# uc-vision/taichi-splatting

Hardware: AMD Instinct MI355X
Metric: fwd+bwd Msplats/s (higher is better)
Workload: dtype f32; 1 GPU; config D: 6000000 random 3D gaussians, 2048x2048, SH deg 3, tile 16, fwd+bwd (render_gaussians, loss=image.sum()); n_gaussians=6000000, tile_size=16, sh_degree=3, mode=single, parallelism=single GPU

## Files before the change

### include/mi355_splat.h

```cpp
#ifndef MI355_SPLAT_H
#define MI355_SPLAT_H

#include <stddef.h>
#include <stdint.h>

#ifdef __cplusplus
extern "C" {
#endif

#define MS_VERSION 500
#define MS_ABI_GENERATION(version) ((version) / 100)

enum { MS_F32 = 0, MS_F64 = 1 };

enum {
  MS_ERR_BAD_ARG = -1,
  MS_ERR_UNSUPPORTED = -2,
  MS_ERR_TMP_TOO_SMALL = -3,
  MS_ERR_ABI = -4
};

typedef struct ms_raster_config {
  int32_t tile_size;
  int32_t antialias;
// ... 134 lines not shown
  uint32_t abi_version;
  int64_t n;
  int64_t k_capacity;
  int32_t image_w, image_h;
  int32_t dtype;
  int32_t f;
  int32_t sh_degree;
  int32_t depth16;
  int32_t tile_row_begin, tile_row_end;
  int32_t projected_input;
  int32_t mapper;
  int32_t split_long_runs;
  int32_t split_seg_len;
  double near_plane, far_plane, blur_cov, clamp_margin;
  ms_raster_config raster;
} ms_frame_desc;

typedef struct ms_frame_layout {
  size_t keep_n_bytes, scratch_n_bytes, keep_k_bytes, scratch_k_bytes;
  size_t points7, depth, colours, points7_f32, camera_position, counters, tile_ranges;
  size_t sorted_keys, order, counts, cum, ordered_points, tmp_n;
  size_t overlap_to_point;
  size_t keys, values, keys_sorted, tmp_k;
  size_t splat_rows;
  size_t split_scratch;
} ms_frame_layout;

typedef struct ms_frame_inputs {
  uint32_t struct_size;
  uint32_t reserved;
  const void *position, *log_scaling, *rotation, *alpha_logit, *feature, *T_camera_world, *projection;
  const void *points7, *depth, *colours;
  int32_t* longest_run_host;
  void* colours_ready_event;
} ms_frame_inputs;

enum { MS_BACKWARD_ALL = 0, MS_BACKWARD_GAUSSIANS = 1, MS_BACKWARD_RASTER = 2 };

typedef struct ms_frame_grads {
  uint32_t struct_size;
// ... 107 lines not shown
```

### taichi_splatting_amd/_lib.py

```python
from __future__ import annotations

import ctypes
from ctypes import c_int, c_int32, c_int64, c_double, c_float, c_void_p, c_size_t, c_char_p, POINTER
import os
from pathlib import Path
import subprocess
from typing import Optional

import torch

PACKAGE_DIR = Path(__file__).resolve().parent
CSRC_DIR = PACKAGE_DIR / 'csrc'
LIB_PATH = Path(os.environ.get('MS_SPLAT_LIB') or PACKAGE_DIR / 'libmi355_splat.so')

MS_F32, MS_F64 = 0, 1
BACKWARD_ALL, BACKWARD_GAUSSIANS, BACKWARD_RASTER = 0, 1, 2
BOUNDARY_AXIS_SIGMA, BOUNDARY_COVARIANCE = 0, 1
MAPPER_DIRECT, MAPPER_PRESORT = 0, 1
ABI_VERSION = 500
MOMENT_ROW = 16
SPLAT_ROW = 16

_lib: Optional[ctypes.CDLL] = None

# ... 20 lines not shown
    self.struct_size = ctypes.sizeof(type(self))
    if hasattr(self, 'abi_version'):
      self.abi_version = ABI_VERSION


class FrameDescC(_SizedStructure):
  _fields_ = [
    ('struct_size', ctypes.c_uint32), ('abi_version', ctypes.c_uint32),
    ('n', c_int64), ('k_capacity', c_int64),
    ('image_w', c_int32), ('image_h', c_int32),
    ('dtype', c_int32), ('f', c_int32), ('sh_degree', c_int32), ('depth16', c_int32),
    ('tile_row_begin', c_int32), ('tile_row_end', c_int32),
    ('projected_input', c_int32), ('mapper', c_int32), ('split_long_runs', c_int32), ('split_seg_len', c_int32),
    ('near_plane', c_double), ('far_plane', c_double), ('blur_cov', c_double), ('clamp_margin', c_double),
    ('raster', RasterConfigC),
  ]


class FrameLayoutC(ctypes.Structure):
  _fields_ = [(name, c_size_t) for name in (
    'keep_n_bytes', 'scratch_n_bytes', 'keep_k_bytes', 'scratch_k_bytes',
    'points7', 'depth', 'colours', 'points7_f32', 'camera_position', 'counters', 'tile_ranges',
    'sorted_keys', 'order', 'counts', 'cum', 'ordered_points', 'tmp_n',
    'overlap_to_point',
    'keys', 'values', 'keys_sorted', 'tmp_k',
    'splat_rows', 'split_scratch')]


class FrameInputsC(_SizedStructure):
  _fields_ = [('struct_size', ctypes.c_uint32), ('reserved', ctypes.c_uint32)] + [(name, c_void_p) for name in (
    'position', 'log_scaling', 'rotation', 'alpha_logit', 'feature', 'T_camera_world', 'projection',
    'points7', 'depth', 'colours', 'longest_run_host', 'colours_ready_event')]


class FrameGradsC(_SizedStructure):
  _fields_ = [
    ('struct_size', ctypes.c_uint32), ('reserved', ctypes.c_uint32),
    ('image', c_void_p), ('grad_image', c_void_p),
    ('extra_points7', c_void_p), ('extra_depth', c_void_p), ('extra_colours', c_void_p),
    ('moments', c_void_p), ('deterministic', c_int32), ('stage', c_int32), ('fixed_exp', c_void_p),
    ('grad_points7', c_void_p), ('grad_colours', c_void_p),
# ... 159 lines not shown
```

### taichi_splatting_amd/csrc/frame.hip

```cpp
#include <cstdlib>
#include <cstring>
#include "common.h"
#include "frame_internal.h"
#include "raster_common.h"

namespace ms {

struct FrameGeom {
  int w_pad, h_pad, tiles_wide, tiles_high, num_tiles, tile_bits, row_begin, row_end;
  size_t es;
};

static FrameGeom frame_geom(const ms_frame_desc* d) {
  FrameGeom g;
  const int ts = d->raster.tile_size;
  g.tiles_wide = (d->image_w + ts - 1) / ts;
  g.tiles_high = (d->image_h + ts - 1) / ts;
  g.w_pad = g.tiles_wide * ts;
  g.h_pad = g.tiles_high * ts;
  g.num_tiles = g.tiles_wide * g.tiles_high;
  int bits = 1;
  while ((1ll << bits) < (long long)g.num_tiles) ++bits;
  g.tile_bits = bits;
  g.row_begin = d->tile_row_begin < 0 ? 0 : d->tile_row_begin;
// ... 24 lines not shown
  if (d->depth16) {
    const FrameGeom g = frame_geom(d);
    if (g.num_tiles > 65536) { set_error("%s: use_depth16 keys hold a 16 bit tile id: too many tiles", who); return MS_ERR_BAD_ARG; }
  }
  return 0;
}

static bool frame_uses_rows(const ms_frame_desc* d) {
  static const bool on = [] { const char* e = getenv("MS_SPLAT_ROWS"); return e && e[0] == '1'; }();
  return on && !d->projected_input && d->n > 0 && raster_uses_splat_rows(&d->raster, d->f, d->dtype);
}

static bool frame_uses_split(const ms_frame_desc* d) {
  return d->split_long_runs != 0 && d->n > 0 && d->k_capacity > 0 && raster_uses_splat_rows(&d->raster, d->f, d->dtype);
}
static SplitParams frame_split_params(const ms_frame_desc* d) {
  return split_params(d->raster.tile_size, d->split_long_runs, d->split_seg_len);
}

static int check_inputs(const ms_frame_inputs* in, const char* who) {
  if (!in) { set_error("%s: inputs are null", who); return MS_ERR_BAD_ARG; }
  if (in->struct_size != sizeof(ms_frame_inputs)) {
    set_error("%s: ms_frame_inputs of another ABI (struct_size %u, this library: %u)", who, in->struct_size, (unsigned)sizeof(ms_frame_inputs));
    return MS_ERR_ABI;
  }
  return 0;
}

static int check_grads(const ms_frame_grads* g, const char* who) {
  if (!g) { set_error("%s: grads are null", who); return MS_ERR_BAD_ARG; }
// ... 23 lines not shown
  L->splat_rows = keep_n.take(frame_uses_rows(d) ? n * SPLAT_ROW * sizeof(float) : 0);
  L->keep_n_bytes = keep_n.off;

  L->sorted_keys = scratch_n.take(n * 4);
  L->order = scratch_n.take(n * 4);
  L->counts = scratch_n.take(n * 4);
  L->cum = scratch_n.take((n + 1) * 4);
  L->ordered_points = scratch_n.take(n * 7 * 4);
  L->points7_f32 = scratch_n.take(d->dtype == MS_F64 ? n * 7 * 4 : 0);
  const size_t t1 = sort_tmp_size(d->n, 4, true), t2 = scan_tmp_size(d->n);
  L->tmp_n = scratch_n.take(t1 > t2 ? t1 : t2);
  L->scratch_n_bytes = scratch_n.off;

  L->overlap_to_point = keep_k.take(k * 4);
  L->split_scratch = keep_k.take(frame_uses_split(d) ? split_scratch_bytes(d->k_capacity, d->raster.tile_size, frame_split_params(d)) : 0);
  L->keep_k_bytes = keep_k.off;

  L->keys = scratch_k.take(k * 8);
  L->values = scratch_k.take(k * 4);
  L->keys_sorted = scratch_k.take(k * 8);
  L->tmp_k = scratch_k.take(sort_tmp_size(d->k_capacity, 8));
  L->scratch_k_bytes = scratch_k.off;
}

template <typename T>
__global__ void __launch_bounds__(256)
frame_prepare_kernel(int32_t* __restrict__ counters, int32_t capacity, const T* __restrict__ Tcw, T* __restrict__ cam_out,
                     int32_t* __restrict__ ranges, int64_t range_words) {
  const int64_t i = (int64_t)blockIdx.x * blockDim.x + threadIdx.x;
  if (i < range_words) ranges[i] = 0;
// ... 221 lines not shown
      const int64_t strip_tiles = (int64_t)(g.row_end > g.row_begin ? g.row_end - g.row_begin : 0) * g.tiles_wide;
      tile_depth_sort_launch(ranges + 2 * first_tile, strip_tiles, keys_sorted, o2p, keys, s, counters + 3, in->longest_run_host);
    }
  }
  MS_CHECK_LAUNCH();

  const void* points7 = d.projected_input ? in->points7 : (const void*)(kn + L.points7);
  const void* colours = d.sh_degree >= 0 ? (const void*)(kn + L.colours) : (d.projected_input ? in->colours : in->feature);
  MS_CHECK_ARG(d.n == 0 || colours != nullptr, "colours are null");
  SplitScratch split{};
  const bool cut = frame_uses_split(desc) && keep_k != nullptr;
  if (cut) split = split_scratch_carve(kk + L.split_scratch, d.k_capacity, d.raster.tile_size, frame_split_params(desc));
  if (in->colours_ready_event) MS_CHECK_HIP(hipStreamWaitEvent(s, (hipEvent_t)in->colours_ready_event, 0));
  return raster_fwd_launch(points7, colours, frame_uses_rows(desc) ? (const float*)(kn + L.splat_rows) : nullptr, ranges, o2p,
                           d.image_w, d.image_h, d.f, &d.raster, out_image, out_alpha, out_visibility, g.row_begin, g.row_end,
                           d.dtype, stream, cut ? &split : nullptr, in->longest_run_host);
}

extern "C" int ms_frame_backward(const ms_frame_desc* desc, const ms_frame_inputs* in, void* keep_n, void* keep_k,
                                 const ms_frame_grads* gr, void* stream) {
  MS_TRY(check_desc(desc, "ms_frame_backward"));
  MS_TRY(check_inputs(in, "ms_frame_backward"));
  MS_TRY(check_grads(gr, "ms_frame_backward"));
  MS_CHECK_ARG(in && keep_n && gr, "null pointer");
  MS_CHECK_ARG(gr->stage == MS_BACKWARD_GAUSSIANS || (gr->image && gr->grad_image), "null image / grad_image");
  const ms_frame_desc& d = *desc;
  const FrameGeom g = frame_geom(desc);
  ms_frame_layout L;
  frame_layout(desc, &L);
  hipStream_t s = (hipStream_t)stream;
  char* kn = (char*)keep_n;
// ... 20 lines not shown
    MS_CHECK_ARG(!d.projected_input, "projected input has no per-gaussian backward");
    if (gr->gather_world > 0)
      MS_CHECK_ARG(gr->gather_rows && gr->gather_slots && gr->gather_route && gr->boundary_stride >= 7 + d.f && d.dtype == MS_F32,
                   "gathered boundary gradients: rows, slots, route, boundary_stride >= 7 + f, float32");
    else
      MS_CHECK_ARG(gr->grad_points7 != nullptr, "grad_points7 is null");
  } else if (moments) {
    MS_CHECK_ARG(gr->moments != nullptr, "moments is null");
    SplitScratch split{};
    const bool cut = frame_uses_split(desc) && keep_k != nullptr;
    if (cut) split = split_scratch_carve(kk + L.split_scratch, d.k_capacity, d.raster.tile_size, frame_split_params(desc));
    MS_TRY(raster_bwd_moments_launch(points7, colours, ranges, o2p, gr->image, gr->grad_image, d.image_w, d.image_h, &d.raster,
                                     (float*)gr->moments, gr->deterministic, gr->fixed_exp, g.row_begin, g.row_end,
                                     gr->grad_image_broadcast, s,
                                     frame_uses_rows(desc) ? (const float*)(kn + L.splat_rows) : nullptr,
                                     cut ? &split : nullptr));
    if (raster_only)
      return moments_finalize_rezero_launch((const float*)points7, (float*)gr->moments, gr->deterministic, gr->fixed_exp,
                                            d.n, (float*)gr->grad_points7, (float*)gr->grad_colours,
                                            d.raster.compute_point_heuristic ? (float*)gr->point_heuristic : nullptr, s,
                                            gr->boundary_stride, d.projected_input && gr->stage != MS_BACKWARD_RASTER ? 0 : gr->boundary_form);
  } else {
    MS_CHECK_ARG(gr->grad_points7 || gr->grad_colours, "no gradient accumulator");
    MS_TRY(ms_raster_bwd(points7, colours, ranges, o2p, gr->image, gr->grad_image, d.image_w, d.image_h, d.f, &d.raster,
                         gr->grad_points7, gr->grad_colours, d.raster.compute_point_heuristic ? gr->point_heuristic : nullptr,
                         g.row_begin, g.row_end, d.dtype, stream));
    if (raster_only) return 0;
  }

  GaussianBwdArgs a{};
  a.dtype = d.dtype;
// ... 28 lines not shown
```

### taichi_splatting_amd/csrc/frame_internal.h

```cpp
#pragma once
#include "common.h"

namespace ms {

constexpr uint32_t CULLED_DEPTH_KEY = 0xffffffffu;

template <typename T>
__device__ inline void camera_position_solve(const T* __restrict__ m, T* __restrict__ out) {
#pragma clang fp contract(off)
  double a[4][5];
  for (int r = 0; r < 4; ++r) {
    for (int c = 0; c < 4; ++c) a[r][c] = (double)m[r * 4 + c];
    a[r][4] = r == 3 ? 1.0 : 0.0;
  }
  for (int col = 0; col < 4; ++col) {
    int piv = col;
    for (int r = col + 1; r < 4; ++r)
      if (fabs(a[r][col]) > fabs(a[piv][col])) piv = r;
    for (int c = 0; c < 5; ++c) { const double t = a[col][c]; a[col][c] = a[piv][c]; a[piv][c] = t; }
    const double inv = 1.0 / a[col][col];
    for (int c = 0; c < 5; ++c) a[col][c] *= inv;
    for (int r = 0; r < 4; ++r) {
      if (r == col) continue;
      const double fct = a[r][col];
// ... 39 lines not shown
                            uint64_t* scratch, hipStream_t s, int32_t* run_stats = nullptr, int32_t* run_host = nullptr);

int project_fwd_launch(const void* position, const void* log_scaling, const void* rotation, const void* alpha_logit,
                       const void* T_camera_world, const void* projection, int image_w, int image_h, double near_plane,
                       double far_plane, double blur_cov, double clamp_margin, double alpha_threshold, int64_t n,
                       void* out_points7, void* out_depth, int32_t* out_flag, int dtype, void* stream, float* splat_rows,
                       const void* colours_in);

int sh_fwd_inplace_launch(const void* params, const void* positions, const void* depth, const void* cam_pos,
                          int64_t n, int f, int degree, void* out, int dtype, hipStream_t s, float* splat_rows = nullptr);

bool raster_uses_splat_rows(const ms_raster_config* cfg, int f, int dtype);
int raster_fwd_launch(const void* points7, const void* features, const float* splat_rows, const int32_t* tile_ranges,
                      const int32_t* overlap_to_point, int image_w, int image_h, int f, const ms_raster_config* cfg,
                      void* out_image, void* out_alpha, void* out_visibility, int tile_row_begin, int tile_row_end,
                      int dtype, void* stream, const struct SplitScratch* split = nullptr, int32_t* long_run_word = nullptr);

int raster_bwd_moments_launch(const void* points7, const void* features, const int32_t* tile_ranges,
                              const int32_t* overlap_to_point, const void* image, const void* grad_image, int image_w,
                              int image_h, const ms_raster_config* cfg, float* moments, int deterministic,
                              const int32_t* fixed_exp, int tile_row_begin, int tile_row_end, int grad_broadcast,
                              hipStream_t s, const float* splat_rows = nullptr, const struct SplitScratch* split = nullptr);
int moments_finalize_rezero_launch(const float* points7, float* moments, int deterministic, const int32_t* fixed_exp,
                                   int64_t n, float* grad_points7, float* grad_features, float* point_heuristic,
                                   hipStream_t s, int row_stride = 0, int covariance_form = 0);

struct FastParams;
bool launch_rows_backward(const float* points7, const float* features, const int32_t* tile_ranges,
                          const int32_t* overlap_to_point, const float* image, const float* grad_image,
                          const FastParams& rp, int tile_size, bool heuristics, float* moments, const int32_t* fixed_exp,
                          hipStream_t s);

struct GaussianBwdArgs {
  int dtype;
  int64_t n;
  const void *position, *log_scaling, *rotation, *alpha_logit, *T_camera_world, *projection;
  int image_w, image_h;
// ... 26 lines not shown
```

### taichi_splatting_amd/csrc/raster.hip

```cpp
#include <stdlib.h>
#include <string.h>

#include "raster_common.h"
#include "frame_internal.h"

namespace ms {

constexpr int RASTER_MAX_F = 4;
constexpr int RASTER_MAX_F_HEUR = 16;
template <int F> struct GradSlots { static constexpr int N = F <= 4 ? 16 : 7 + F + 2; };

template <typename T> struct RasterParams {
  int width, height, tiles_wide, tile_begin;
  T clamp_max_alpha, alpha_threshold, saturate_threshold;
};

template <typename T, int F> struct alignas(16) Splat {
  T mx, my, A, B;
  T C, D, isx, isy;
  T alpha;
  T f[F];
  T ax, ay, sx, sy;
};
template <typename T> struct CullBox { T cx, cy, ex, ey; };
// ... 456 lines not shown
  switch (ts) {
    case 8: launch_bwd<T, F, 8>(args...); return 0;
    case 16: launch_bwd<T, F, 16>(args...); return 0;
    case 32: launch_bwd<T, F, 32>(args...); return 0;
  }
  return MS_ERR_UNSUPPORTED;
}

}

using namespace ms;

bool ms_raster_fwd_fast(const void* points, const void* feats, const int32_t* ranges, const int32_t* o2p,
                        int w, int h, const ms_raster_config* cfg, void* image, void* alpha, void* visibility,
                        int row_begin, int num_tiles, hipStream_t s, const float* splat_rows, const SplitScratch* split,
                        int32_t* long_run_word);
bool ms_raster_bwd_fast(const void* points, const void* feats, const int32_t* ranges, const int32_t* o2p,
                        const void* image, const void* grad_image, int w, int h, const ms_raster_config* cfg,
                        void* gp, void* gf, void* heur, int row_begin, int num_tiles, hipStream_t s);

static int check_raster_common(const ms_raster_config* cfg, int w, int h, int f, int dtype, int* row_begin,
                               int* row_end, const char* fn, int max_f = RASTER_MAX_F) {
  if (!cfg) { set_error("%s: cfg is null", fn); return MS_ERR_BAD_ARG; }
  if (w <= 0 || h <= 0) { set_error("%s: bad image size %dx%d", fn, w, h); return MS_ERR_BAD_ARG; }
  if (dtype != MS_F32 && dtype != MS_F64) { set_error("%s: dtype must be MS_F32 or MS_F64", fn); return MS_ERR_BAD_ARG; }
  if (cfg->tile_size != 8 && cfg->tile_size != 16 && cfg->tile_size != 32) {
    set_error("%s: tile_size must be 8, 16 or 32 (got %d)", fn, cfg->tile_size); return MS_ERR_UNSUPPORTED;
  }
  if (f < 1 || f > max_f || (f > RASTER_MAX_F && f != 8 && f != 16)) {
    set_error("%s: feature size %d not supported: 1..%d, or 8 / 16 for the backward pass with point heuristics "
              "(split or zero-pad the channels on the host)", fn, f, RASTER_MAX_F);
// ... 73 lines not shown
    set_error("ms_raster_fwd_rows: splat rows serve float32 RGB, plain pdf, alpha blending, tile 8 / 16 / 32");
    return MS_ERR_UNSUPPORTED;
  }
  return raster_fwd_launch(rows, rows, rows, tile_ranges, overlap_to_point, image_w, image_h, 3, cfg, out_image, out_alpha,
                           out_visibility, tile_row_begin, tile_row_end, MS_F32, stream);
}

bool ms::raster_uses_splat_rows(const ms_raster_config* cfg, int f, int dtype) {
  return dtype == MS_F32 && f == 3 && !cfg->antialias && cfg->use_alpha_blending &&
         (cfg->tile_size == 8 || cfg->tile_size == 16 || cfg->tile_size == 32);
}

int ms::raster_fwd_launch(const void* points7, const void* features, const float* splat_rows, const int32_t* tile_ranges,
                      const int32_t* overlap_to_point, int image_w, int image_h, int f, const ms_raster_config* cfg,
                      void* out_image, void* out_alpha, void* out_visibility, int tile_row_begin, int tile_row_end,
                      int dtype, void* stream, const SplitScratch* split, int32_t* long_run_word) {
  int rc = check_raster_common(cfg, image_w, image_h, f, dtype, &tile_row_begin, &tile_row_end, "ms_raster_fwd");
  if (rc) return rc;
  MS_CHECK_ARG(tile_ranges && out_image && out_alpha, "null pointer");
  if (tile_row_end <= tile_row_begin) return 0;
  const int tiles_wide = (image_w + cfg->tile_size - 1) / cfg->tile_size;
  const int num_tiles = (tile_row_end - tile_row_begin) * tiles_wide;
  hipStream_t s = (hipStream_t)stream;
  if (dtype == MS_F32 && f == 3 && !cfg->antialias && cfg->use_alpha_blending) {
    void* vis = (cfg->compute_visibility && out_visibility) ? out_visibility : nullptr;
    if (ms_raster_fwd_fast(points7, features, tile_ranges, overlap_to_point, image_w, image_h, cfg, out_image,
                           out_alpha, vis, tile_row_begin, num_tiles, s, splat_rows, split, long_run_word)) {
      MS_CHECK_LAUNCH();
      return 0;
    }
  }
#define MS_GO(T, F) rc = dispatch_ts_fwd<T, F>(cfg->tile_size, points7, features, tile_ranges, overlap_to_point, image_w, image_h, cfg, out_image, out_alpha, out_visibility, tile_row_begin, num_tiles, s)
  if (dtype == MS_F32) {
    switch (f) { case 1: MS_GO(float, 1); break; case 2: MS_GO(float, 2); break; case 3: MS_GO(float, 3); break; default: MS_GO(float, 4); break; }
  } else {
    switch (f) { case 1: MS_GO(double, 1); break; case 2: MS_GO(double, 2); break; case 3: MS_GO(double, 3); break; default: MS_GO(double, 4); break; }
  }
#undef MS_GO
  if (rc) return rc;
  MS_CHECK_LAUNCH();
  return 0;
}
// ... 45 lines not shown
```

### taichi_splatting_amd/csrc/raster_bwd_scan.hip

```cpp
#include <stdlib.h>

#include <type_traits>

#include "raster_bwd_shared.h"
#include "frame_internal.h"

#ifndef MS_SCAN_STATS
#define MS_SCAN_STATS 0
#endif
#ifndef MS_SCAN_ABLATE
#define MS_SCAN_ABLATE 0
#endif
#ifndef MS_SCAN_PHASES
#define MS_SCAN_PHASES 0
#endif
#ifndef MS_COMMIT_ABLATE
#define MS_COMMIT_ABLATE 0
#endif
#ifndef MS_PRIO_MODE
#define MS_PRIO_MODE 1
#endif
#if MS_PRIO_MODE == 1
#define MS_PRIO_BLEND(on) __builtin_amdgcn_s_setprio((on) ? 2 : 0)
#elif MS_PRIO_MODE == 2
// ... 121 lines not shown
  const float oms = rp.one_minus_saturate;
  const uint32_t oms_bits = __float_as_uint(oms);

  for (int i = lane; i < CAP * NACC; i += 64) (&s_acc[wave][0][0])[i] = 0.0f;

  const int start = SEGS ? seg_start : ranges[tile_id * 2 + 0], end = SEGS ? seg_end : ranges[tile_id * 2 + 1];
  if (end <= start) return;
  if (!SEGS && rp.split_min_run > 0 && end - start > rp.split_min_run && rp.split_counts[2] == 0) return;

  const int total = end - start;
  int num_batches = (total + BATCH_TARGET / 2) / BATCH_TARGET;
  if (num_batches < 1) num_batches = 1;
  int bsz = (total + num_batches - 1) / num_batches;
  if (bsz > BATCH) { num_batches = (total + BATCH - 1) / BATCH; bsz = (total + num_batches - 1) / num_batches; }

  Raw raw = {};
  int next_id = 0;
  ScanRecord rec = {};
  int rec_id = 0;
  auto list_pos = [&](int j, int sl) { const int i = start + j * bsz + sl; return i < end ? i : end - 1; };
  constexpr int B_THREADS = 16 * SLOTS_B;
  static_assert(B_THREADS <= THREADS, "one lane per component of the extra slots");
  const int b_slot = PRIMARY + ((t >> 4) < (SLOTS_B > 0 ? SLOTS_B : 1) ? (t >> 4) : 0), b_comp = t & 15;
  const bool b_lane = SLOTS_B > 0 && t < B_THREADS && b_comp <= 10;
  float b_val = 0.0f, b_hold = 0.0f;
  int b_nid = 0;
  const bool b_geom = b_comp < 7, b_col = b_comp >= 7 && b_comp < 10;
  auto b_load = [&](int id, int j) {
    const uint64_t pa = reinterpret_cast<uint64_t>(points), fa = reinterpret_cast<uint64_t>(feats),
                   oa = reinterpret_cast<uint64_t>(o2p);
    const int g_row = ROWS ? SPLAT_ROW : 7, c_row = ROWS ? SPLAT_ROW : 3, c_off = ROWS ? SPLAT_ROW_COLOUR : 0;
    const uint64_t a_geom = pa + 4ull * (uint64_t)((int64_t)id * g_row + (b_geom ? b_comp : 0));
    const uint64_t a_col = (ROWS ? pa : fa) + 4ull * (uint64_t)((int64_t)id * c_row + c_off + (b_col ? b_comp - 7 : 0));
    const uint64_t a_id = oa + 4ull * (uint64_t)list_pos(j, b_slot);
    uint64_t addr = b_geom ? a_geom : (b_col ? a_col : a_id);
    asm volatile("" : "+v"(addr));
    return *reinterpret_cast<const __attribute__((address_space(1))) float*>(addr);
  };
  if (PIPELINED) {
    next_id = o2p[list_pos(0, t)];
    if (SLOTS_B > 0) b_nid = o2p[list_pos(0, b_slot)];
  }
  auto stage_next = [&](int batch) {
    if (!PIPELINED) return;
    if (batch + 1 >= 0 && batch + 1 < num_batches) { rec = make_scan_record(raw, rp.alpha_threshold); rec_id = raw.id; }
    else { rec = ScanRecord{}; rec_id = 0; }
    asm volatile("" : "+v"(rec.r0.x), "+v"(rec.r0.y), "+v"(rec.r0.z), "+v"(rec.r0.w), "+v"(rec.r1.x), "+v"(rec.r1.y),
                      "+v"(rec.r1.z), "+v"(rec.r1.w), "+v"(rec.r2.x), "+v"(rec.r2.y), "+v"(rec.r2.z), "+v"(rec.r2.w), "+v"(rec_id));
    __builtin_amdgcn_sched_barrier(0);
    int gather_id;
    asm volatile("v_mov_b32 %0, %1" : "=v"(gather_id) : "v"(next_id));
    raw = load_raw<ROWS>(points, feats, gather_id);
    next_id = o2p[list_pos(batch + 3, t)];
    if (SLOTS_B > 0) {
      asm volatile("v_mov_b32 %0, %1" : "=v"(b_hold) : "v"(b_val));
      b_val = b_load(b_nid, batch + 2);
      b_nid = o2p[list_pos(batch + 3, b_slot)];
    }
  };

#if MS_SCAN_STATS
  __shared__ int s_bsum, s_bmax;
  if (t == 0) { s_bsum = 0; s_bmax = 0; }
#define MS_FLUSH_BALANCE()                                                                                      \
  if (t == 0) {                                                                                                 \
    atomicAdd(&g_scan_stats[8], (unsigned long long)s_bsum);                                                    \
    atomicAdd(&g_scan_stats[9], (unsigned long long)(s_bmax * WAVES));                                          \
// ... 471 lines not shown
  static const bool q = [] { const char* e = getenv("MS_TILE32_BWD"); return e && e[0] == 'q'; }();
  return q;
}

static hipEvent_t g_probe_start = nullptr, g_probe_stop = nullptr;
extern "C" int ms_probe_raster_bwd(void* start_event, void* stop_event) {
  g_probe_start = (hipEvent_t)start_event; g_probe_stop = (hipEvent_t)stop_event;
  return 0;
}

static int launch_scan_backward(const float* points7, const float* features,
                                const int32_t* tile_ranges, const int32_t* overlap_to_point, const float* image,
                                const float* grad_image, int image_w, int image_h, const ms_raster_config* cfg,
                                float* moments, int deterministic, const int32_t* fixed_exp, int tile_row_begin,
                                int tile_row_end, hipStream_t s, const char* who, int grad_broadcast = 0,
                                const float* splat_rows = nullptr, const SplitScratch* split = nullptr) {
  if (deterministic && !fixed_exp) { set_error("%s: deterministic commits need fixed_exp (ms_fixed_point_exponents)", who); return MS_ERR_BAD_ARG; }
  if (image_w <= 0 || image_h <= 0) { set_error("%s: bad image size", who); return MS_ERR_BAD_ARG; }
  if (!cfg->use_alpha_blending) {
    set_error("%s: backward requires use_alpha_blending (reference: tests/test_rasterizer.py:92-94)", who);
    return MS_ERR_BAD_ARG;
  }
  if (cfg->antialias) { set_error("%s: antialiased pdf is served by ms_raster_bwd", who); return MS_ERR_UNSUPPORTED; }
  const int ts = cfg->tile_size;
  if (ts != 8 && ts != 16 && ts != 32) { set_error("%s: tile_size must be 8, 16 or 32 (got %d)", who, ts); return MS_ERR_UNSUPPORTED; }
  const int tiles_high = (image_h + ts - 1) / ts, tiles_wide = (image_w + ts - 1) / ts;
  if (tile_row_begin < 0) tile_row_begin = 0;
  if (tile_row_end > tiles_high) tile_row_end = tiles_high;
  if (tile_row_end <= tile_row_begin) return 0;

  FastParams rp{};
  rp.width = image_w; rp.height = image_h; rp.tiles_wide = tiles_wide; rp.tile_begin = tile_row_begin * tiles_wide;
  rp.clamp_max_alpha = (float)cfg->clamp_max_alpha;
  rp.alpha_threshold = (float)cfg->alpha_threshold;
  rp.one_minus_saturate = (float)(1.0 - cfg->saturate_threshold);
  rp.deterministic = deterministic != 0;
  rp.grad_broadcast = grad_broadcast != 0;
  rp.num_tiles = (tile_row_end - tile_row_begin) * tiles_wide;
  if (split && ts == 32 && tile32_quarters()) split = nullptr;
  if (split) {
    rp.split_min_run = split->min_run;
    rp.split_items = split->items; rp.split_counts = split->counts; rp.split_state = split->state;
  }
#define MS_GO(TS, HEUR, SPLIT, ROWS) raster_bwd_scan_kernel<TS, HEUR, SPLIT, ROWS>                               \
      <<<dim3(xcd_grid<(SPLIT > 1 ? 1 : 0)>(rp.num_tiles, SPLIT * SPLIT)), dim3(TS * TS), 0, s>>>(              \
          ROWS ? splat_rows : points7, features, tile_ranges, overlap_to_point, image, grad_image, rp, moments, fixed_exp)
#define MS_GO_TILE(TS, SPLIT, ROWS)                                                                             \
  do { if (hf) MS_GO(TS, true, SPLIT, ROWS); else MS_GO(TS, false, SPLIT, ROWS); } while (0)
#define MS_GO_SEGS(TS)                                                                                          \
  do {                                                                                                          \
    if (hf) raster_bwd_scan_kernel<TS, true, 1, false, true><<<dim3((unsigned)split->item_cap), dim3(TS * TS), 0, s>>>(  \
        points7, features, tile_ranges, overlap_to_point, image, grad_image, rp, moments, fixed_exp);          \
    else raster_bwd_scan_kernel<TS, false, 1, false, true><<<dim3((unsigned)split->item_cap), dim3(TS * TS), 0, s>>>(    \
        points7, features, tile_ranges, overlap_to_point, image, grad_image, rp, moments, fixed_exp);          \
// ... 112 lines not shown
  hipStream_t s = (hipStream_t)stream;
#define MS_GO(HEUR, FIXED) raster_moments_finalize_kernel<HEUR, FIXED><<<grid, 256, 0, s>>>(            \
      (const float*)points7, const_cast<float*>(moments), n, grad_points7, grad_features, point_heuristic, fixed_exp)
  if (point_heuristic) { if (deterministic) MS_GO(true, true); else MS_GO(true, false); }
  else { if (deterministic) MS_GO(false, true); else MS_GO(false, false); }
#undef MS_GO
  MS_CHECK_LAUNCH();
  return 0;
}

namespace ms {
int raster_bwd_moments_launch(const void* points7, const void* features, const int32_t* tile_ranges,
                              const int32_t* overlap_to_point, const void* image, const void* grad_image, int image_w,
                              int image_h, const ms_raster_config* cfg, float* moments, int deterministic,
                              const int32_t* fixed_exp, int tile_row_begin, int tile_row_end, int grad_broadcast,
                              hipStream_t s, const float* splat_rows, const SplitScratch* split) {
  return launch_scan_backward((const float*)points7, (const float*)features, tile_ranges, overlap_to_point,
                              (const float*)image, (const float*)grad_image, image_w, image_h, cfg, moments,
                              deterministic, fixed_exp, tile_row_begin, tile_row_end, s, "ms_frame_backward", grad_broadcast,
                              splat_rows, split);
}

int moments_finalize_rezero_launch(const float* points7, float* moments, int deterministic, const int32_t* fixed_exp,
                                   int64_t n, float* grad_points7, float* grad_features, float* point_heuristic,
                                   hipStream_t s, int row_stride, int covariance_form) {
  if (n == 0) return 0;
  const dim3 grid((unsigned)div_up(n, 256));
  const int gp_stride = row_stride > 0 ? row_stride : 7, gf_stride = row_stride > 0 ? row_stride : 3;
#define MS_GO(HEUR, FIXED) raster_moments_finalize_kernel<HEUR, FIXED, true><<<grid, 256, 0, s>>>(      \
      points7, moments, n, grad_points7, grad_features, point_heuristic, fixed_exp, gp_stride, gf_stride, covariance_form)
  if (point_heuristic) { if (deterministic) MS_GO(true, true); else MS_GO(true, false); }
  else { if (deterministic) MS_GO(false, true); else MS_GO(false, false); }
#undef MS_GO
  MS_CHECK_LAUNCH();
  return 0;
// ... 3 lines not shown
```

### taichi_splatting_amd/csrc/raster_common.h

```cpp
#pragma once
#include <stdlib.h>
#include "common.h"

namespace ms {

struct FastParams {
  int width, height, tiles_wide, tile_begin;
  float clamp_max_alpha, alpha_threshold, one_minus_saturate;
  int deterministic;
  int num_tiles;
  int grad_broadcast;
  int split_min_run;
  const int4* split_items;
  const int32_t* split_counts;
  float4* split_state;
  int32_t* long_run_word;
};

constexpr int SPLIT_MIN_RUN = 16384;
constexpr int SPLIT_MAX_SEG = 256;
static inline int split_default_seg_len(int tile_size) {
  static const int forced = [] { const char* e = getenv("MS_SPLIT_SEG"); const int v = e ? atoi(e) : 0; return v >= 256 ? (v + 255) & ~255 : 0; }();
  if (forced) return forced;
  return tile_size == 32 ? 4096 : 1024;
}
struct SplitParams { int min_run, seg_len; };
static inline SplitParams split_params(int tile_size, int min_run_req, int seg_req) {
  SplitParams sp;
  sp.min_run = min_run_req > 1 ? (min_run_req < 256 ? 256 : min_run_req) : SPLIT_MIN_RUN;
  sp.seg_len = seg_req > 0 ? ((seg_req + 255) & ~255) : split_default_seg_len(tile_size);
  return sp;
// ... 39 lines not shown
  }
}
template <unsigned CHUNK>
static inline unsigned xcd_grid(int num_tiles, unsigned parts) {
  if (CHUNK == 0) return (unsigned)num_tiles * parts;
  const unsigned span = NUM_XCD * CHUNK;
  return ((unsigned)num_tiles + span - 1) / span * span * parts;
}

struct Raw {
  float g[7];
  float f[3];
  int id;
};

template <bool ROWS = false>
__device__ __forceinline__ Raw load_raw(const float* __restrict__ points, const float* __restrict__ feats, int id) {
  Raw r;
  if constexpr (ROWS) {
    const float4* row = reinterpret_cast<const float4*>(points) + (int64_t)id * (SPLAT_ROW / 4);
    const float4 a = row[0], b = row[1], c = row[2];
    r.g[0] = a.x; r.g[1] = a.y; r.g[2] = a.z; r.g[3] = a.w; r.g[4] = b.x; r.g[5] = b.y; r.g[6] = b.z;
    r.f[0] = c.x; r.f[1] = c.y; r.f[2] = c.z;
  } else {
    const float* g = points + (int64_t)id * 7;
    const float* f = feats + (int64_t)id * 3;
#pragma unroll
    for (int k = 0; k < 7; ++k) r.g[k] = g[k];
#pragma unroll
    for (int k = 0; k < 3; ++k) r.f[k] = f[k];
  }
  r.id = id;
  return r;
}

#ifndef MS_SLOW_STAGING
#define MS_SLOW_STAGING 0
#endif
#if MS_SLOW_STAGING
__device__ __forceinline__ float rcp_newton(float x) { return 1.0f / x; }
__device__ __forceinline__ float stage_rcp(float x) { return 1.0f / x; }
__device__ __forceinline__ float fast_sqrt(float x) { return sqrtf(x); }
__device__ __forceinline__ float fast_log2(float x) { return log2f(x); }
#else
__device__ __forceinline__ float rcp_newton(float x) {
  const float r = __builtin_amdgcn_rcpf(x);
// ... 131 lines not shown
```

### taichi_splatting_amd/csrc/raster_fast.hip

```cpp
#include "raster_common.h"

#ifndef MS_ABLATE
#define MS_ABLATE 0
#endif
#ifndef MS_FWD_PHASES
#define MS_FWD_PHASES 0
#endif
#ifndef MS_FWD_CLAMP_FOLD
#define MS_FWD_CLAMP_FOLD 1
#endif
#ifndef MS_FWD_SKIP_EMPTY
#define MS_FWD_SKIP_EMPTY 0
#endif
#ifndef MS_FWD_PAIR
#define MS_FWD_PAIR 1
#endif

namespace ms {

#if MS_FWD_PHASES
__device__ unsigned long long* g_fwd_phase_rows = nullptr;
#define MS_FPH(i) do { const uint64_t ph_now = __builtin_readcyclecounter(); ph_acc[i] += (uint32_t)(ph_now - ph_last); ph_last = ph_now; } while (0)
#else
#define MS_FPH(i) do {} while (0)
// ... 6 lines not shown
#define FWD_ALPHA_BIAS (__builtin_amdgcn_logf(rp.clamp_max_alpha))
__device__ __forceinline__ float fwd_alpha(float e, float) { return __builtin_amdgcn_fmed3f(e, 0.0f, 1.0f); }
#else
#define FWD_ALPHA_BIAS 0.0f
__device__ __forceinline__ float fwd_alpha(float e, float clamp_max_alpha) { return clamp_alpha(e, clamp_max_alpha); }
#endif

template <int TS, bool VIS, bool ROWS, bool SEGS = false>
__global__ void __launch_bounds__(TS * TS)
raster_fwd_f32x3_kernel(const float* __restrict__ points, const float* __restrict__ feats,
                        const int32_t* __restrict__ ranges, const int32_t* __restrict__ o2p,
                        FastParams rp, float* __restrict__ image, float* __restrict__ image_alpha,
                        float* __restrict__ visibility) {
  using G = TileGeom<TS>;
  constexpr int BATCH = G::BATCH;
  __shared__ float4 s_rec[BATCH * 3];
  __shared__ float4 s_cull[BATCH * 2];
  __shared__ int32_t s_id[VIS ? BATCH : 1];
  __shared__ float s_vis[VIS ? BATCH : 1];
#if MS_FWD_PHASES
  const uint64_t ph_start = __builtin_readcyclecounter();
  uint64_t ph_last = ph_start;
  uint32_t ph_acc[11] = {0, 0, 0, 0, 0, 0, 0, 0, 0, 0, 0};
#endif

  int tile_id, start, end;
  if constexpr (SEGS) {
    if (rp.split_counts[2] != 0 || (int)blockIdx.x >= rp.split_counts[0]) return;
    const int4 item = rp.split_items[blockIdx.x];
    tile_id = item.x; start = item.y; end = item.z;
// ... 24 lines not shown
  const float TSCALE = 1.0f, GATE = rp.alpha_threshold;
#endif
  float T = in_bounds ? TSCALE : 0.0f;
  if constexpr (SEGS && VIS) T = TSCALE * rp.split_state[(int64_t)blockIdx.x * (TS * TS) + threadIdx.x].w;
  const float SPENT = FWD_SPENT_T * TSCALE;

  const int t = threadIdx.x;

  Raw raw;
  int next_id = 0;
  const bool stager = t < BATCH;
  if (stager && start + t < end) raw = load_raw<ROWS>(points, feats, o2p[start + t]);
  if (stager && start + BATCH + t < end) next_id = o2p[start + BATCH + t];
  if (VIS && stager) s_vis[t] = 0.0f;

  for (int begin = start; begin < end; begin += BATCH) {
    const int count = (end - begin) < BATCH ? (end - begin) : BATCH;
    if (begin == start) MS_FPH(7);
    const bool wave_spent = __ballot(T >= SPENT) == 0;
    if (lane == 0) reinterpret_cast<int*>(&s_rec[wave * 3 + 2])[3] = wave_spent ? 1 : 0;
    __syncthreads();
    if (__ballot(reinterpret_cast<const int*>(&s_rec[(lane % (TS * TS / 64)) * 3 + 2])[3] != 0) == ~0ull) break;
    MS_FPH(0);
    if (VIS && stager) {
      if (begin > start && s_vis[t] != 0.0f) atomic_add_noret(visibility + s_id[t], s_vis[t]);
      s_vis[t] = 0.0f;
    }
    MS_FPH(5);
    if (stager && begin + t < end) {
      write_records<true>(raw, rp.alpha_threshold, &s_rec[t * 3], &s_cull[t * 2], origin_x, origin_y, FWD_ALPHA_BIAS);
      if (VIS) s_id[t] = raw.id;
    }
    if (stager && begin + BATCH + t < end) raw = load_raw<ROWS>(points, feats, next_id);
    if (stager && begin + 2 * BATCH + t < end) next_id = o2p[begin + 2 * BATCH + t];
    MS_FPH(1);
    __syncthreads();
    MS_FPH(2);
#if MS_FWD_PHASES
    ph_acc[10] += 1;
#endif
    if (wave_spent) continue;

    for (int r = 0; r < count; r += 64) {
      const int j = r + lane;
      bool hit = false;
      if (j < count) hit = patch_hit(s_cull[j * 2], s_cull[j * 2 + 1], rcx, rcy);
// ... 67 lines not shown
        const float Y = __builtin_fmaf(pxr, q1.x, __builtin_fmaf(pyr, q1.y, -q0.y));
        const float a = fwd_alpha(__builtin_amdgcn_exp2f(-__builtin_fmaf(Y, Y, __builtin_fmaf(X, X, q1.z))), rp.clamp_max_alpha);
        const bool pass = a > GATE;
#if MS_FWD_SKIP_EMPTY
        if (__ballot(pass) == 0) continue;
        const float2 q2 = *reinterpret_cast<const float2*>(&s_rec[(r + b) * 3 + 2]);
#endif
        const float w = pass ? a * T : 0.0f;
        T = __builtin_fmaf(-TSCALE, w, T);
        c0 += q1.w * w; c1 += q2.x * w; c2 += q2.y * w;
      }
      MS_FPH(4);
    }
  }
  MS_FPH(6);

  if (VIS && end > start) {
    __syncthreads();
    if (stager && s_vis[t] != 0.0f) atomic_add_noret(visibility + s_id[t], s_vis[t]);
  }

#if MS_FWD_CLAMP_FOLD
  T = T / TSCALE;
#endif
#if MS_FWD_PHASES
  if (g_fwd_phase_rows && lane == 0) {
    unsigned long long* row = g_fwd_phase_rows + ((size_t)blockIdx.x * (TS * TS / 64) + wave) * 12;
    const uint64_t now = __builtin_readcyclecounter();
    ph_acc[6] += (uint32_t)(now - ph_last);
    for (int i = 0; i < 8; ++i) row[i] = ph_acc[i];
// ... 220 lines not shown
  rp.width = w; rp.height = h;
  rp.tiles_wide = (w + cfg->tile_size - 1) / cfg->tile_size;
  rp.tile_begin = row_begin * rp.tiles_wide;
  rp.clamp_max_alpha = (float)cfg->clamp_max_alpha;
  rp.alpha_threshold = (float)cfg->alpha_threshold;
  rp.one_minus_saturate = (float)(1.0 - cfg->saturate_threshold);
  rp.deterministic = 0;
  rp.num_tiles = num_tiles;
  rp.grad_broadcast = 0;
  return rp;
}

bool ms_raster_fwd_fast(const void* points, const void* feats, const int32_t* ranges, const int32_t* o2p,
                        int w, int h, const ms_raster_config* cfg, void* image, void* alpha, void* visibility,
                        int row_begin, int num_tiles, hipStream_t s, const float* splat_rows, const SplitScratch* split,
                        int32_t* long_run_word) {
  FastParams rp = make_fast_params(w, h, cfg, row_begin, num_tiles);
  rp.long_run_word = long_run_word;
  const bool cut = split != nullptr;
  if (cut) {
    rp.split_min_run = split->min_run;
    rp.split_items = split->items; rp.split_counts = split->counts; rp.split_state = split->state;
    (void)hipMemsetAsync(split->counts, 0, 4 * sizeof(int32_t), s);
    split_plan_kernel<<<dim3((unsigned)((num_tiles + 255) / 256)), dim3(256), 0, s>>>(
        ranges, rp.tile_begin, num_tiles, split->min_run, split->seg_len, (int)split->item_cap, (int)split->long_cap,
        split->counts, split->long_tiles, split->items);
  }
  const dim3 grid(xcd_grid<FWD_XCD_CHUNK>(rp.num_tiles, 1));
#define MS_GO3(TS, VIS, ROWS)                                                                                   \
  raster_fwd_f32x3_kernel<TS, VIS, ROWS><<<grid, dim3(TS * TS), 0, s>>>(                                        \
      ROWS ? splat_rows : (const float*)points, (const float*)feats, ranges, o2p, rp, (float*)image, (float*)alpha,  \
      VIS ? (float*)visibility : nullptr)
#define MS_SEG(TS, VIS, ROWS)                                                                                   \
// ... 43 lines not shown
```

### taichi_splatting_amd/frame.py

```python
from __future__ import annotations

import collections
import contextlib
import ctypes
import gc
from dataclasses import dataclass, replace
import os
import threading
import time
from typing import Optional, Tuple
import weakref

import torch

from . import _lib
from .data_types import RasterConfig

USE_FRAME = os.environ.get('MS_FRAME', 'frame') != 'legacy'

K_SLACK = 1.25
K_GRANULE = 1 << 16

_k_capacity = {}
_mapper_mode = {}
PRESORT_ABOVE, DIRECT_BELOW = 3.6, 3.4
LONG_RUN_LIMIT = 16384
_run_words = {}
_presort_sticky = set()
_k_host = {}
_moments = collections.OrderedDict()
_moments_pinned = set()
_identity = {}
_lock = threading.RLock()

MOMENTS_LRU = 4
K_SLOTS = 64
GRAPH_K_WORDS = 1024
SPLIT_LONG_RUNS = os.environ.get('MS_SPLIT_LONG_RUNS', '1') not in ('', '0')
SPLIT_MIN_RUN = int(os.environ.get('MS_SPLIT_MIN_RUN', '0'))
SPLIT_SEG_LEN = int(os.environ.get('MS_SPLIT_SEG_LEN', '0'))
SPLIT_ALWAYS = os.environ.get('MS_SPLIT_ALWAYS', '0') not in ('', '0')
BROADCAST_GRAD = os.environ.get('MS_BROADCAST_GRAD', '1') not in ('', '0')
STRICT = os.environ.get('MS_STRICT', '0') not in ('', '0')

LAZY_SETTLE = os.environ.get('MS_LAZY_SETTLE', '0') not in ('', '0')
VISIBILITY_FROM_BACKWARD = os.environ.get('MS_VISIBILITY_FROM_BACKWARD', '0') not in ('', '0')
SH_SIDE_STREAM = os.environ.get('MS_SH_SIDE_STREAM', '1') not in ('', '0')
_side_streams = {}
visibility_passes = 0
LAZY_AFTER = 3
_stable_frames = {}
_unsettled = collections.deque()

# ... 524 lines not shown
      f, d = feat.shape[1], feat.shape[2]
      degree = int(round(d ** 0.5)) - 1
      assert (degree + 1) ** 2 == d, f"SH feature count must be square, got {d} ({feat.shape})"
      assert 0 <= degree <= 3, f"SH degree must be between 0 and 3, got {degree}"
    else:
      assert feat.ndim == 2, f"Features must be (N, C) if use_sh=False, got {feat.shape}"
      f, degree = feat.shape[1], -1

    rows = (0, tiles_high) if opts.tile_rows is None else (max(0, int(opts.tile_rows[0])), min(tiles_high, int(opts.tile_rows[1])))
    key = _shape_key(device, n, (w, h), config, opts.tile_rows, opts.use_depth16)
    desc = _lib.FrameDescC(n=n, k_capacity=_k_capacity.get(key, 0), image_w=w, image_h=h, dtype=_lib.dtype_code(dtype), f=f,
                           sh_degree=degree, depth16=int(opts.use_depth16), tile_row_begin=rows[0], tile_row_end=rows[1],
                           projected_input=0, mapper=0, near_plane=float(opts.depth_range[0]),
                           far_plane=float(opts.depth_range[1]), blur_cov=float(config.blur_cov),
                           clamp_margin=float(config.clamp_margin), raster=_lib.raster_config_c(config))
    layout = _lib.FrameLayoutC()
    _lib.check(lib.ms_frame_layout_query(ctypes.byref(desc), ctypes.byref(layout)), "render_gaussians")
    stream = _lib.current_stream(device)
    keep_n = torch.empty((layout.keep_n_bytes,), dtype=torch.uint8, device=device)
    scratch_n = torch.empty((layout.scratch_n_bytes,), dtype=torch.uint8, device=device)
    inputs = _lib.FrameInputsC(position=pos.data_ptr(), log_scaling=lsc.data_ptr(), rotation=rot.data_ptr(),
                               alpha_logit=alog.data_ptr(), feature=feat.data_ptr(), T_camera_world=Tcw.data_ptr(),
                               projection=proj.data_ptr(), points7=None, depth=None, colours=None)

    y0, y1 = _strip_pixels(rows, ts, h) if opts.crop_to_rows else (0, h)
    image = torch.empty((y1 - y0, w, f), dtype=dtype, device=device)
    alpha = torch.empty((y1 - y0, w), dtype=dtype, device=device)
    if not opts.crop_to_rows and rows != (0, tiles_high):
      image.zero_(); alpha.zero_()
    visibility = torch.zeros((n,), dtype=dtype, device=device) if config.compute_visibility else torch.empty((0,), dtype=dtype, device=device)
# ... 382 lines not shown
```

Baseline: 1991 Msplats/s.

## Cache per-overlap gathered splat rows in forward for sequential backward reads

```diff
diff --git a/include/mi355_splat.h b/include/mi355_splat.h
--- a/include/mi355_splat.h
+++ b/include/mi355_splat.h
@@ -172,6 +172,8 @@
   int32_t split_seg_len;
   double near_plane, far_plane, blur_cov, clamp_margin;
   ms_raster_config raster;
+  int32_t list_rows;
+  int32_t reserved2;
 } ms_frame_desc;
 
 typedef struct ms_frame_layout {
@@ -182,6 +184,7 @@
   size_t keys, values, keys_sorted, tmp_k;
   size_t splat_rows;
   size_t split_scratch;
+  size_t list_rows;
 } ms_frame_layout;
 
 typedef struct ms_frame_inputs {
diff --git a/taichi_splatting_amd/_lib.py b/taichi_splatting_amd/_lib.py
--- a/taichi_splatting_amd/_lib.py
+++ b/taichi_splatting_amd/_lib.py
@@ -58,6 +58,7 @@
     ('projected_input', c_int32), ('mapper', c_int32), ('split_long_runs', c_int32), ('split_seg_len', c_int32),
     ('near_plane', c_double), ('far_plane', c_double), ('blur_cov', c_double), ('clamp_margin', c_double),
     ('raster', RasterConfigC),
+    ('list_rows', c_int32), ('reserved2', c_int32),
   ]
 
 
@@ -68,7 +69,7 @@
     'sorted_keys', 'order', 'counts', 'cum', 'ordered_points', 'tmp_n',
     'overlap_to_point',
     'keys', 'values', 'keys_sorted', 'tmp_k',
-    'splat_rows', 'split_scratch')]
+    'splat_rows', 'split_scratch', 'list_rows')]
 
 
 class FrameInputsC(_SizedStructure):
diff --git a/taichi_splatting_amd/csrc/frame.hip b/taichi_splatting_amd/csrc/frame.hip
--- a/taichi_splatting_amd/csrc/frame.hip
+++ b/taichi_splatting_amd/csrc/frame.hip
@@ -62,6 +62,10 @@
 static bool frame_uses_split(const ms_frame_desc* d) {
   return d->split_long_runs != 0 && d->n > 0 && d->k_capacity > 0 && raster_uses_splat_rows(&d->raster, d->f, d->dtype);
 }
+static bool frame_uses_list_rows(const ms_frame_desc* d) {
+  return d->list_rows != 0 && d->n > 0 && d->k_capacity > 0 && d->raster.tile_size == 16 && !frame_uses_rows(d) &&
+         raster_uses_splat_rows(&d->raster, d->f, d->dtype);
+}
 static SplitParams frame_split_params(const ms_frame_desc* d) {
   return split_params(d->raster.tile_size, d->split_long_runs, d->split_seg_len);
 }
@@ -115,6 +119,7 @@
 
   L->overlap_to_point = keep_k.take(k * 4);
   L->split_scratch = keep_k.take(frame_uses_split(d) ? split_scratch_bytes(d->k_capacity, d->raster.tile_size, frame_split_params(d)) : 0);
+  L->list_rows = keep_k.take(frame_uses_list_rows(d) ? k * LIST_ROW * sizeof(float) : 0);
   L->keep_k_bytes = keep_k.off;
 
   L->keys = scratch_k.take(k * 8);
@@ -366,7 +371,8 @@
   if (in->colours_ready_event) MS_CHECK_HIP(hipStreamWaitEvent(s, (hipEvent_t)in->colours_ready_event, 0));
   return raster_fwd_launch(points7, colours, frame_uses_rows(desc) ? (const float*)(kn + L.splat_rows) : nullptr, ranges, o2p,
                            d.image_w, d.image_h, d.f, &d.raster, out_image, out_alpha, out_visibility, g.row_begin, g.row_end,
-                           d.dtype, stream, cut ? &split : nullptr, in->longest_run_host);
+                           d.dtype, stream, cut ? &split : nullptr, in->longest_run_host,
+                           frame_uses_list_rows(desc) ? (float*)(kk + L.list_rows) : nullptr);
 }
 
 extern "C" int ms_frame_backward(const ms_frame_desc* desc, const ms_frame_inputs* in, void* keep_n, void* keep_k,
@@ -417,7 +423,8 @@
                                      (float*)gr->moments, gr->deterministic, gr->fixed_exp, g.row_begin, g.row_end,
                                      gr->grad_image_broadcast, s,
                                      frame_uses_rows(desc) ? (const float*)(kn + L.splat_rows) : nullptr,
-                                     cut ? &split : nullptr));
+                                     cut ? &split : nullptr,
+                                     frame_uses_list_rows(desc) && keep_k ? (const float*)(kk + L.list_rows) : nullptr));
     if (raster_only)
       return moments_finalize_rezero_launch((const float*)points7, (float*)gr->moments, gr->deterministic, gr->fixed_exp,
                                             d.n, (float*)gr->grad_points7, (float*)gr->grad_colours,
diff --git a/taichi_splatting_amd/csrc/frame_internal.h b/taichi_splatting_amd/csrc/frame_internal.h
--- a/taichi_splatting_amd/csrc/frame_internal.h
+++ b/taichi_splatting_amd/csrc/frame_internal.h
@@ -77,13 +77,15 @@
 int raster_fwd_launch(const void* points7, const void* features, const float* splat_rows, const int32_t* tile_ranges,
                       const int32_t* overlap_to_point, int image_w, int image_h, int f, const ms_raster_config* cfg,
                       void* out_image, void* out_alpha, void* out_visibility, int tile_row_begin, int tile_row_end,
-                      int dtype, void* stream, const struct SplitScratch* split = nullptr, int32_t* long_run_word = nullptr);
+                      int dtype, void* stream, const struct SplitScratch* split = nullptr, int32_t* long_run_word = nullptr,
+                      float* list_rows = nullptr);
 
 int raster_bwd_moments_launch(const void* points7, const void* features, const int32_t* tile_ranges,
                               const int32_t* overlap_to_point, const void* image, const void* grad_image, int image_w,
                               int image_h, const ms_raster_config* cfg, float* moments, int deterministic,
                               const int32_t* fixed_exp, int tile_row_begin, int tile_row_end, int grad_broadcast,
-                              hipStream_t s, const float* splat_rows = nullptr, const struct SplitScratch* split = nullptr);
+                              hipStream_t s, const float* splat_rows = nullptr, const struct SplitScratch* split = nullptr,
+                              const float* list_rows = nullptr);
 int moments_finalize_rezero_launch(const float* points7, float* moments, int deterministic, const int32_t* fixed_exp,
                                    int64_t n, float* grad_points7, float* grad_features, float* point_heuristic,
                                    hipStream_t s, int row_stride = 0, int covariance_form = 0);
diff --git a/taichi_splatting_amd/csrc/raster.hip b/taichi_splatting_amd/csrc/raster.hip
--- a/taichi_splatting_amd/csrc/raster.hip
+++ b/taichi_splatting_amd/csrc/raster.hip
@@ -494,7 +494,7 @@
 bool ms_raster_fwd_fast(const void* points, const void* feats, const int32_t* ranges, const int32_t* o2p,
                         int w, int h, const ms_raster_config* cfg, void* image, void* alpha, void* visibility,
                         int row_begin, int num_tiles, hipStream_t s, const float* splat_rows, const SplitScratch* split,
-                        int32_t* long_run_word);
+                        int32_t* long_run_word, float* list_rows = nullptr);
 bool ms_raster_bwd_fast(const void* points, const void* feats, const int32_t* ranges, const int32_t* o2p,
                         const void* image, const void* grad_image, int w, int h, const ms_raster_config* cfg,
                         void* gp, void* gf, void* heur, int row_begin, int num_tiles, hipStream_t s);
@@ -598,7 +598,7 @@
 int ms::raster_fwd_launch(const void* points7, const void* features, const float* splat_rows, const int32_t* tile_ranges,
                       const int32_t* overlap_to_point, int image_w, int image_h, int f, const ms_raster_config* cfg,
                       void* out_image, void* out_alpha, void* out_visibility, int tile_row_begin, int tile_row_end,
-                      int dtype, void* stream, const SplitScratch* split, int32_t* long_run_word) {
+                      int dtype, void* stream, const SplitScratch* split, int32_t* long_run_word, float* list_rows) {
   int rc = check_raster_common(cfg, image_w, image_h, f, dtype, &tile_row_begin, &tile_row_end, "ms_raster_fwd");
   if (rc) return rc;
   MS_CHECK_ARG(tile_ranges && out_image && out_alpha, "null pointer");
@@ -609,7 +609,7 @@
   if (dtype == MS_F32 && f == 3 && !cfg->antialias && cfg->use_alpha_blending) {
     void* vis = (cfg->compute_visibility && out_visibility) ? out_visibility : nullptr;
     if (ms_raster_fwd_fast(points7, features, tile_ranges, overlap_to_point, image_w, image_h, cfg, out_image,
-                           out_alpha, vis, tile_row_begin, num_tiles, s, splat_rows, split, long_run_word)) {
+                           out_alpha, vis, tile_row_begin, num_tiles, s, splat_rows, split, long_run_word, list_rows)) {
       MS_CHECK_LAUNCH();
       return 0;
     }
diff --git a/taichi_splatting_amd/csrc/raster_bwd_scan.hip b/taichi_splatting_amd/csrc/raster_bwd_scan.hip
--- a/taichi_splatting_amd/csrc/raster_bwd_scan.hip
+++ b/taichi_splatting_amd/csrc/raster_bwd_scan.hip
@@ -159,6 +159,9 @@
   int bsz = (total + num_batches - 1) / num_batches;
   if (bsz > BATCH) { num_batches = (total + BATCH - 1) / BATCH; bsz = (total + num_batches - 1) / num_batches; }
 
+  constexpr bool LIST_ROWS_OK = TS == 16 && SPLIT == 1 && !ROWS;
+  const bool list_rows = LIST_ROWS_OK && rp.list_rows != nullptr;
+  const uint64_t la = reinterpret_cast<uint64_t>(rp.list_rows);
   Raw raw = {};
   int next_id = 0;
   ScanRecord rec = {};
@@ -175,9 +178,13 @@
     const uint64_t pa = reinterpret_cast<uint64_t>(points), fa = reinterpret_cast<uint64_t>(feats),
                    oa = reinterpret_cast<uint64_t>(o2p);
     const int g_row = ROWS ? SPLAT_ROW : 7, c_row = ROWS ? SPLAT_ROW : 3, c_off = ROWS ? SPLAT_ROW_COLOUR : 0;
-    const uint64_t a_geom = pa + 4ull * (uint64_t)((int64_t)id * g_row + (b_geom ? b_comp : 0));
-    const uint64_t a_col = (ROWS ? pa : fa) + 4ull * (uint64_t)((int64_t)id * c_row + c_off + (b_col ? b_comp - 7 : 0));
-    const uint64_t a_id = oa + 4ull * (uint64_t)list_pos(j, b_slot);
+    const int pos = list_pos(j, b_slot);
+    const uint64_t g_base = list_rows ? la : pa, c_base = list_rows ? la : (ROWS ? pa : fa);
+    const int g_str = list_rows ? LIST_ROW : g_row, c_str = list_rows ? LIST_ROW : c_row, c_o = list_rows ? 7 : c_off;
+    const int row = list_rows ? pos : id;
+    const uint64_t a_geom = g_base + 4ull * (uint64_t)((int64_t)row * g_str + (b_geom ? b_comp : 0));
+    const uint64_t a_col = c_base + 4ull * (uint64_t)((int64_t)row * c_str + c_o + (b_col ? b_comp - 7 : 0));
+    const uint64_t a_id = oa + 4ull * (uint64_t)pos;
     uint64_t addr = b_geom ? a_geom : (b_col ? a_col : a_id);
     asm volatile("" : "+v"(addr));
     return *reinterpret_cast<const __attribute__((address_space(1))) float*>(addr);
@@ -195,7 +202,15 @@
     __builtin_amdgcn_sched_barrier(0);
     int gather_id;
     asm volatile("v_mov_b32 %0, %1" : "=v"(gather_id) : "v"(next_id));
-    raw = load_raw<ROWS>(points, feats, gather_id);
+    if constexpr (LIST_ROWS_OK) {
+      const uint64_t g_base = list_rows ? la : reinterpret_cast<uint64_t>(points);
+      const uint64_t f_base = list_rows ? la + 28ull : reinterpret_cast<uint64_t>(feats);
+      const uint64_t g_str = list_rows ? 4ull * LIST_ROW : 28ull, f_str = list_rows ? 4ull * LIST_ROW : 12ull;
+      const int64_t row = list_rows ? (int64_t)list_pos(batch + 2, t) : (int64_t)gather_id;
+      raw = load_raw_global(g_base + g_str * (uint64_t)row, f_base + f_str * (uint64_t)row, gather_id);
+    } else {
+      raw = load_raw<ROWS>(points, feats, gather_id);
+    }
     next_id = o2p[list_pos(batch + 3, t)];
     if (SLOTS_B > 0) {
       asm volatile("v_mov_b32 %0, %1" : "=v"(b_hold) : "v"(b_val));
@@ -697,7 +712,8 @@
                                 const float* grad_image, int image_w, int image_h, const ms_raster_config* cfg,
                                 float* moments, int deterministic, const int32_t* fixed_exp, int tile_row_begin,
                                 int tile_row_end, hipStream_t s, const char* who, int grad_broadcast = 0,
-                                const float* splat_rows = nullptr, const SplitScratch* split = nullptr) {
+                                const float* splat_rows = nullptr, const SplitScratch* split = nullptr,
+                                const float* list_rows = nullptr) {
   if (deterministic && !fixed_exp) { set_error("%s: deterministic commits need fixed_exp (ms_fixed_point_exponents)", who); return MS_ERR_BAD_ARG; }
   if (image_w <= 0 || image_h <= 0) { set_error("%s: bad image size", who); return MS_ERR_BAD_ARG; }
   if (!cfg->use_alpha_blending) {
@@ -721,6 +737,7 @@
   rp.grad_broadcast = grad_broadcast != 0;
   rp.num_tiles = (tile_row_end - tile_row_begin) * tiles_wide;
   if (split && ts == 32 && tile32_quarters()) split = nullptr;
+  rp.list_rows = ts == 16 && !splat_rows ? const_cast<float*>(list_rows) : nullptr;
   if (split) {
     rp.split_min_run = split->min_run;
     rp.split_items = split->items; rp.split_counts = split->counts; rp.split_state = split->state;
@@ -863,11 +880,12 @@
                               const int32_t* overlap_to_point, const void* image, const void* grad_image, int image_w,
                               int image_h, const ms_raster_config* cfg, float* moments, int deterministic,
                               const int32_t* fixed_exp, int tile_row_begin, int tile_row_end, int grad_broadcast,
-                              hipStream_t s, const float* splat_rows, const SplitScratch* split) {
+                              hipStream_t s, const float* splat_rows, const SplitScratch* split,
+                              const float* list_rows) {
   return launch_scan_backward((const float*)points7, (const float*)features, tile_ranges, overlap_to_point,
                               (const float*)image, (const float*)grad_image, image_w, image_h, cfg, moments,
                               deterministic, fixed_exp, tile_row_begin, tile_row_end, s, "ms_frame_backward", grad_broadcast,
-                              splat_rows, split);
+                              splat_rows, split, list_rows);
 }
 
 int moments_finalize_rezero_launch(const float* points7, float* moments, int deterministic, const int32_t* fixed_exp,
diff --git a/taichi_splatting_amd/csrc/raster_common.h b/taichi_splatting_amd/csrc/raster_common.h
--- a/taichi_splatting_amd/csrc/raster_common.h
+++ b/taichi_splatting_amd/csrc/raster_common.h
@@ -15,6 +15,7 @@
   const int32_t* split_counts;
   float4* split_state;
   int32_t* long_run_word;
+  float* list_rows;
 };
 
 constexpr int SPLIT_MIN_RUN = 16384;
@@ -84,6 +85,19 @@
   int id;
 };
 
+constexpr int LIST_ROW = 10;
+__device__ __forceinline__ void store_list_row(const Raw& r, float* __restrict__ dst) {
+#pragma unroll
+  for (int k = 0; k < 7; ++k) dst[k] = r.g[k];
+#pragma unroll
+  for (int k = 0; k < 3; ++k) dst[7 + k] = r.f[k];
+}
+__device__ __forceinline__ void store_null_list_row(float* __restrict__ dst) {
+  dst[0] = __builtin_nanf(""); dst[1] = __builtin_nanf("");
+#pragma unroll
+  for (int k = 2; k < LIST_ROW; ++k) dst[k] = 0.0f;
+}
+
 template <bool ROWS = false>
 __device__ __forceinline__ Raw load_raw(const float* __restrict__ points, const float* __restrict__ feats, int id) {
   Raw r;
@@ -100,6 +114,19 @@
 #pragma unroll
     for (int k = 0; k < 3; ++k) r.f[k] = f[k];
   }
+  r.id = id;
+  return r;
+}
+
+__device__ __forceinline__ Raw load_raw_global(uint64_t g, uint64_t f, int id) {
+  using gfloat = const __attribute__((address_space(1))) float;
+  gfloat* gp = reinterpret_cast<gfloat*>(g);
+  gfloat* fp = reinterpret_cast<gfloat*>(f);
+  Raw r;
+#pragma unroll
+  for (int k = 0; k < 7; ++k) r.g[k] = gp[k];
+#pragma unroll
+  for (int k = 0; k < 3; ++k) r.f[k] = fp[k];
   r.id = id;
   return r;
 }
diff --git a/taichi_splatting_amd/csrc/raster_fast.hip b/taichi_splatting_amd/csrc/raster_fast.hip
--- a/taichi_splatting_amd/csrc/raster_fast.hip
+++ b/taichi_splatting_amd/csrc/raster_fast.hip
@@ -44,6 +44,7 @@
                         float* __restrict__ visibility) {
   using G = TileGeom<TS>;
   constexpr int BATCH = G::BATCH;
+  constexpr bool LIST_ROWS = TS == 16 && !ROWS && !(SEGS && VIS);
   __shared__ float4 s_rec[BATCH * 3];
   __shared__ float4 s_cull[BATCH * 2];
   __shared__ int32_t s_id[VIS ? BATCH : 1];
@@ -98,13 +99,17 @@
   if (stager && start + BATCH + t < end) next_id = o2p[start + BATCH + t];
   if (VIS && stager) s_vis[t] = 0.0f;
 
+  int unstaged = end;
   for (int begin = start; begin < end; begin += BATCH) {
     const int count = (end - begin) < BATCH ? (end - begin) : BATCH;
     if (begin == start) MS_FPH(7);
     const bool wave_spent = __ballot(T >= SPENT) == 0;
     if (lane == 0) reinterpret_cast<int*>(&s_rec[wave * 3 + 2])[3] = wave_spent ? 1 : 0;
     __syncthreads();
-    if (__ballot(reinterpret_cast<const int*>(&s_rec[(lane % (TS * TS / 64)) * 3 + 2])[3] != 0) == ~0ull) break;
+    if (__ballot(reinterpret_cast<const int*>(&s_rec[(lane % (TS * TS / 64)) * 3 + 2])[3] != 0) == ~0ull) {
+      unstaged = begin;
+      break;
+    }
     MS_FPH(0);
     if (VIS && stager) {
       if (begin > start && s_vis[t] != 0.0f) atomic_add_noret(visibility + s_id[t], s_vis[t]);
@@ -114,6 +119,7 @@
     if (stager && begin + t < end) {
       write_records<true>(raw, rp.alpha_threshold, &s_rec[t * 3], &s_cull[t * 2], origin_x, origin_y, FWD_ALPHA_BIAS);
       if (VIS) s_id[t] = raw.id;
+      if (LIST_ROWS && rp.list_rows) store_list_row(raw, rp.list_rows + (int64_t)(begin + t) * LIST_ROW);
     }
     if (stager && begin + BATCH + t < end) raw = load_raw<ROWS>(points, feats, next_id);
     if (stager && begin + 2 * BATCH + t < end) next_id = o2p[begin + 2 * BATCH + t];
@@ -211,6 +217,8 @@
     }
   }
   MS_FPH(6);
+  if (LIST_ROWS && rp.list_rows)
+    for (int i = unstaged + t; i < end; i += TS * TS) store_null_list_row(rp.list_rows + (int64_t)i * LIST_ROW);
 
   if (VIS && end > start) {
     __syncthreads();
@@ -461,9 +469,10 @@
 bool ms_raster_fwd_fast(const void* points, const void* feats, const int32_t* ranges, const int32_t* o2p,
                         int w, int h, const ms_raster_config* cfg, void* image, void* alpha, void* visibility,
                         int row_begin, int num_tiles, hipStream_t s, const float* splat_rows, const SplitScratch* split,
-                        int32_t* long_run_word) {
+                        int32_t* long_run_word, float* list_rows) {
   FastParams rp = make_fast_params(w, h, cfg, row_begin, num_tiles);
   rp.long_run_word = long_run_word;
+  rp.list_rows = cfg->tile_size == 16 && !splat_rows ? list_rows : nullptr;
   const bool cut = split != nullptr;
   if (cut) {
     rp.split_min_run = split->min_run;
diff --git a/taichi_splatting_amd/frame.py b/taichi_splatting_amd/frame.py
--- a/taichi_splatting_amd/frame.py
+++ b/taichi_splatting_amd/frame.py
@@ -37,6 +37,7 @@
 K_SLOTS = 64
 GRAPH_K_WORDS = 1024
 SPLIT_LONG_RUNS = os.environ.get('MS_SPLIT_LONG_RUNS', '1') not in ('', '0')
+LIST_ROWS = os.environ.get('MS_LIST_ROWS', '1') != '0'
 SPLIT_MIN_RUN = int(os.environ.get('MS_SPLIT_MIN_RUN', '0'))
 SPLIT_SEG_LEN = int(os.environ.get('MS_SPLIT_SEG_LEN', '0'))
 SPLIT_ALWAYS = os.environ.get('MS_SPLIT_ALWAYS', '0') not in ('', '0')
@@ -591,6 +592,7 @@
                            projected_input=0, mapper=0, near_plane=float(opts.depth_range[0]),
                            far_plane=float(opts.depth_range[1]), blur_cov=float(config.blur_cov),
                            clamp_margin=float(config.clamp_margin), raster=_lib.raster_config_c(config))
+    desc.list_rows = int(LIST_ROWS and any(ctx.needs_input_grad[:5]))
     layout = _lib.FrameLayoutC()
     _lib.check(lib.ms_frame_layout_query(ctypes.byref(desc), ctypes.byref(layout)), "render_gaussians")
     stream = _lib.current_stream(device)
```

Result: no change. 2011 Msplats/s (median of 6 runs) (+1.0%).
